# spiraldb/vortex

Hardware: AMD Instinct MI355X
Metric: decoded GB/s/GPU (device-resident) per encoding; % HBM roofline (higher is better)
Workload: dtype u32

## Files before the change

### vortex_amd/csrc/capi.hip

```cpp
#include <algorithm>
#include <cstring>
#include <mutex>

#include "encode_gpu.hpp"
#include "planner.hpp"

namespace vxg {

const float kF10f[11] = {1.0f, 10.0f, 100.0f, 1000.0f, 10000.0f, 100000.0f, 1000000.0f,
                         10000000.0f, 100000000.0f, 1000000000.0f, 10000000000.0f};
const float kIF10f[11] = {1.0f, 0.1f, 0.01f, 0.001f, 0.0001f, 0.00001f, 0.000001f,
                          0.0000001f, 0.00000001f, 0.000000001f, 0.0000000001f};
const double kF10d[24] = {
    1.0, 10.0, 100.0, 1000.0, 10000.0, 100000.0, 1000000.0, 10000000.0, 100000000.0,
    1000000000.0, 10000000000.0, 100000000000.0, 1000000000000.0, 10000000000000.0,
    100000000000000.0, 1000000000000000.0, 10000000000000000.0, 100000000000000000.0,
    1000000000000000000.0, 10000000000000000000.0, 100000000000000000000.0,
    1000000000000000000000.0, 10000000000000000000000.0, 100000000000000000000000.0};
const double kIF10d[24] = {
    1.0, 0.1, 0.01, 0.001, 0.0001, 0.00001, 0.000001, 0.0000001, 0.00000001, 0.000000001,
    0.0000000001, 0.00000000001, 0.000000000001, 0.0000000000001, 0.00000000000001,
    0.000000000000001, 0.0000000000000001, 0.00000000000000001, 0.000000000000000001,
    0.0000000000000000001, 0.00000000000000000001, 0.000000000000000000001,
    0.0000000000000000000001, 0.00000000000000000000001};
// ... 94 lines not shown
}

vxg_status vxg_set_option(vxg_ctx* ctx, int option, int64_t value) {
    if (!ctx) return set_error(VXG_ERR_INVALID_ARGUMENT, "null vxg_ctx");
    Options& o = ctx->c.opt;
    switch (option) {
    case VXG_OPT_K1W_MIN_GROUPS:
        if (value < 0 || value > (int64_t(1) << 31)) return set_error(VXG_ERR_INVALID_ARGUMENT, "K1W_MIN_GROUPS out of range");
        o.k1w_min_groups = value;
        return VXG_OK;
    case VXG_OPT_K1W_BPW:
        if (value < 0 || value > 32) return set_error(VXG_ERR_INVALID_ARGUMENT, "K1W_BPW must be in [0, 32]");
        o.k1w_bpw = value;
        return VXG_OK;
    case VXG_OPT_K1_WAVE:
        if (value < -1 || value > 2) return set_error(VXG_ERR_INVALID_ARGUMENT, "K1_WAVE must be -1, 0, 1 or 2");
        o.k1_wave = value;
        return VXG_OK;
    }
    return set_error(VXG_ERR_INVALID_ARGUMENT, "unknown option " + std::to_string(option));
}

vxg_status vxg_get_option(vxg_ctx* ctx, int option, int64_t* value) {
    if (!ctx || !value) return set_error(VXG_ERR_INVALID_ARGUMENT, "null argument");
    const Options& o = ctx->c.opt;
    switch (option) {
    case VXG_OPT_K1W_MIN_GROUPS: *value = o.k1w_min_groups; return VXG_OK;
    case VXG_OPT_K1W_BPW: *value = o.k1w_bpw; return VXG_OK;
    case VXG_OPT_K1_WAVE: *value = o.k1_wave; return VXG_OK;
    }
    return set_error(VXG_ERR_INVALID_ARGUMENT, "unknown option " + std::to_string(option));
}

vxg_status vxg_get_launch_stats(vxg_ctx* ctx, vxg_launch_stats* out, int reset) {
    if (!ctx || !out) return set_error(VXG_ERR_INVALID_ARGUMENT, "null argument");
    std::lock_guard<std::mutex> lk(ctx->c.mu);
    const LaunchStats& st = ctx->c.st;
    *out = vxg_launch_stats{};
    out->k1w_launches = st.k1w_launches;
    out->k1w_last_groups = st.k1w_last_groups;
    out->k1w_last_bpw = st.k1w_last_bpw;
    out->k1w_min_bpw = st.k1w_min_bpw;
    out->k1w_max_bpw = st.k1w_max_bpw;
    out->k1w_last_bpw_max = st.k1w_last_bpw_max;
    if (reset) ctx->c.st = LaunchStats{};
    return VXG_OK;
}

vxg_status vxg_close(vxg_ctx* ctx) {
    if (!ctx) return VXG_OK;
    if (g_cur_ctx == &ctx->c) g_cur_ctx = nullptr;
    (void)hipSetDevice(ctx->c.device);
    (void)hipDeviceSynchronize();
    if (ctx->c.err_word) (void)hipFree(ctx->c.err_word);
    delete ctx;
    return VXG_OK;
}

vxg_status vxg_alloc(vxg_ctx* ctx, uint64_t bytes, void** dptr) {
    VXG_TRY(use_device(ctx));
    return hip_check(hipMalloc(dptr, bytes ? bytes : 16), "hipMalloc");
}

vxg_status vxg_free(vxg_ctx* ctx, void* dptr) {
    VXG_TRY(use_device(ctx));
    return hip_check(hipFree(dptr), "hipFree");
}

vxg_status vxg_host_alloc(vxg_ctx* ctx, uint64_t bytes, void** hptr) {
    VXG_TRY(use_device(ctx));
    return hip_check(hipHostMalloc(hptr, bytes ? bytes : 16, hipHostMallocDefault), "hipHostMalloc");
}

vxg_status vxg_host_free(vxg_ctx* ctx, void* hptr) {
    VXG_TRY(use_device(ctx));
    return hip_check(hipHostFree(hptr), "hipHostFree");
}

vxg_status vxg_memcpy_h2d(vxg_ctx* ctx, void* dst, const void* src, uint64_t bytes, void* stream) {
    VXG_TRY(use_device(ctx));
    return hip_check(hipMemcpyAsync(dst, src, bytes, hipMemcpyHostToDevice, S(stream)), "h2d");
}

vxg_status vxg_memcpy_d2h(vxg_ctx* ctx, void* dst, const void* src, uint64_t bytes, void* stream) {
    VXG_TRY(use_device(ctx));
    return hip_check(hipMemcpyAsync(dst, src, bytes, hipMemcpyDeviceToHost, S(stream)), "d2h");
}

vxg_status vxg_memcpy_d2d(vxg_ctx* ctx, void* dst, const void* src, uint64_t bytes, void* stream) {
    VXG_TRY(use_device(ctx));
    return hip_check(hipMemcpyAsync(dst, src, bytes, hipMemcpyDeviceToDevice, S(stream)), "d2d");
}

vxg_status vxg_stream_sync(vxg_ctx* ctx, void* stream) {
    VXG_TRY(use_device(ctx));
    VXG_TRY(hip_check(hipStreamSynchronize(S(stream)), "hipStreamSynchronize"));
    uint32_t err = 0;
    VXG_TRY(hip_check(hipMemcpy(&err, ctx->c.err_word, 4, hipMemcpyDeviceToHost), "error word readback"));
    if (err) {
        VXG_TRY(hip_check(hipMemset(ctx->c.err_word, 0, 4), "error word reset"));
        return status_of_err_word(err);
    }
    return VXG_OK;
}

vxg_status vxg_canonical_size(vxg_ctx* ctx, const vxg_array* a, uint64_t* values_bytes, uint64_t* data_bytes) {
// ... 500 lines not shown
```

### vortex_amd/csrc/plan.hip

```cpp
#include <algorithm>
#include <chrono>
#include <cstdio>
#include <memory>

#include "k1g.hpp"
#include "planner.hpp"

using namespace vxg;

static uint64_t tree_bytes(const vxg_array& a) {
    uint64_t b = 0;
    for (uint32_t i = 0; i < a.n_buffers; i++) b += a.buffers[i].len;
    for (uint32_t i = 0; i < a.n_children; i++) b += tree_bytes(a.children[i]);
    return b;
}

static uint16_t leading_encoding(const vxg_array& a) {
    return a.encoding == VXG_ENC_CHUNKED && a.n_children ? leading_encoding(a.children[0]) : a.encoding;
}

static uint64_t canonical_out_bytes(const vxg_array& a) {
    return a.dtype == VXG_DTYPE_BOOL ? a.len / 8 : a.len * (is_string(a) ? 16 : ptype_width(a.ptype));
}

// ... 10 lines not shown
}

enum class BatchMode { Auto, Off, On, Mixed, Strings };
static BatchMode plan_batch_mode() {
    const char* e = env_str("VXG_PLAN_BATCH");
    if (!e || !*e) return BatchMode::Auto;
    if (e[0] == '0') return BatchMode::Off;
    if (e[0] == '1') return BatchMode::On;
    if (e[0] == 'm') return BatchMode::Mixed;
    if (e[0] == 's') return BatchMode::Strings;
    return BatchMode::Auto;
}
static bool dict_string_column(const vxg_array& a) {
    if (!is_string(a)) return false;
    if (a.encoding == VXG_ENC_CHUNKED) {
        for (uint32_t i = 1; i < a.n_children; i++)
            if (a.children[i].encoding != VXG_ENC_DICT) return false;
        return a.n_children > 1;
    }
    return a.encoding == VXG_ENC_DICT;
}
static uint64_t plan_batch_max_bytes() { return env_u64("VXG_PLAN_BATCH_MAX_BYTES", uint64_t(64) << 20); }

struct FusedNode {
    FsstFusedArgs fa;
    const GenChunk* gtab;
    uint32_t gn, dict_off;
    bool dict_lds;
    uint32_t* err;
    uint64_t gpe;
    void* args[7];
    hipGraphNode_t node = nullptr;
    hipKernelNodeParams p{};
    explicit FusedNode(void** a) {
        fa = *static_cast<const FsstFusedArgs*>(a[0]);
        gtab = *static_cast<const GenChunk* const*>(a[1]);
        gn = *static_cast<const uint32_t*>(a[2]);
        dict_off = *static_cast<const uint32_t*>(a[3]);
        dict_lds = *static_cast<const bool*>(a[4]);
        err = *static_cast<uint32_t* const*>(a[5]);
        gpe = *static_cast<const uint64_t*>(a[6]);
        void* const mine[7] = {&fa, &gtab, &gn, &dict_off, &dict_lds, &err, &gpe};
        std::copy(mine, mine + 7, args);
    }
};

struct vxg_plan {
    vxg_ctx* ctx = nullptr;
    std::vector<std::unique_ptr<FusedNode>> fused;
    uint64_t launches = 0;
    hipGraph_t graph = nullptr;
    hipGraphExec_t exec = nullptr;
    DevTables store;
    std::vector<hipKernelNodeParams> direct;
    bool batched = false;
    uint32_t branches = 0;
    vxg_plan_info info{};
};

static size_t plan_direct_max() { return size_t(env_u64("VXG_PLAN_DIRECT_MAX", 16)); }
static bool plan_direct_enabled() { return env_flag("VXG_PLAN_DIRECT", true); }

static std::vector<hipKernelNodeParams> kernel_chain(hipGraph_t g) {
    std::vector<hipKernelNodeParams> out;
    size_t nn = 0;
    if (hipGraphGetNodes(g, nullptr, &nn) != hipSuccess || nn == 0 || nn > plan_direct_max()) return out;
    std::vector<hipGraphNode_t> nodes(nn);
    if (hipGraphGetNodes(g, nodes.data(), &nn) != hipSuccess) return out;
    std::vector<hipGraphNode_t> dep(nn, nullptr);
    size_t roots = 0, root = 0;
    for (size_t i = 0; i < nn; i++) {
        hipGraphNodeType t{};
        if (hipGraphNodeGetType(nodes[i], &t) != hipSuccess || t != hipGraphNodeTypeKernel) {
            if (env_str("VXG_PLAN_DEBUG")) std::fprintf(stderr, "plan: node %zu of %zu has type %d\n", i, nn, int(t));
            return out;
        }
        size_t nd = 0;
        if (hipGraphNodeGetDependencies(nodes[i], nullptr, &nd) != hipSuccess || nd > 1) return out;
        if (nd == 1 && hipGraphNodeGetDependencies(nodes[i], &dep[i], &nd) != hipSuccess) return out;
        if (nd == 0) {
            roots++;
            root = i;
        }
    }
    if (roots != 1) return out;
    std::vector<size_t> order{root};
    while (order.size() < nn) {
        size_t next = nn, cnt = 0;
        for (size_t i = 0; i < nn; i++)
            if (dep[i] == nodes[order.back()]) {
                next = i;
                cnt++;
            }
        if (cnt != 1) return out;
        order.push_back(next);
    }
    for (size_t i : order) {
        hipKernelNodeParams p{};
        if (hipGraphKernelNodeGetParams(nodes[i], &p) != hipSuccess || p.extra || !p.kernelParams || !p.func) {
            out.clear();
            return out;
        }
        out.push_back(p);
    }
    return out;
}

static vxg_status bind_fused_nodes(vxg_plan* pl, hipGraph_t g) {
    size_t nn = 0;
    if (hipGraphGetNodes(g, nullptr, &nn) != hipSuccess) return set_error(VXG_ERR_ASSERTION_FAILED, "graph nodes");
    std::vector<hipGraphNode_t> nodes(nn);
    if (nn && hipGraphGetNodes(g, nodes.data(), &nn) != hipSuccess) return set_error(VXG_ERR_ASSERTION_FAILED, "graph nodes");
    for (hipGraphNode_t nd : nodes) {
        hipGraphNodeType t{};
        if (hipGraphNodeGetType(nd, &t) != hipSuccess || t != hipGraphNodeTypeKernel) continue;
        hipKernelNodeParams p{};
        if (hipGraphKernelNodeGetParams(nd, &p) != hipSuccess || !p.kernelParams || !is_fsst_fused_kernel(p.func)) continue;
        if (static_cast<const FsstFusedArgs*>(p.kernelParams[0])->prepass == 0) continue;
        auto f = std::make_unique<FusedNode>(p.kernelParams);
        f->node = nd;
        f->p = p;
        f->p.kernelParams = f->args;
        for (hipKernelNodeParams& d : pl->direct)
            if (d.func == p.func) d.kernelParams = f->args;
        pl->fused.push_back(std::move(f));
    }
    return VXG_OK;
}

static vxg_status record_plan(vxg_ctx* ctx, const vxg_array* arrays, vxg_canonical* outs, uint32_t n,
                              const std::vector<bool>& batched, uint32_t branches, vxg_plan** plan) {
    *plan = nullptr;
    const bool batching = std::find(batched.begin(), batched.end(), true) != batched.end();
    const bool own = batching && branches > 1;
    const uint32_t nb = (n < branches ? (n ? n : 1) : branches) + (own ? 1 : 0);
    const uint32_t na = own ? nb - 1 : nb;
    PlanBatch batch;
    hipStream_t cs;
    VXG_TRY(hip_check(hipStreamCreateWithFlags(&cs, hipStreamNonBlocking), "plan stream"));
    std::vector<hipStream_t> br(nb, nullptr);
    std::vector<hipEvent_t> ev(nb + 1, nullptr);
    vxg_status st = VXG_OK;
    for (uint32_t b = 0; b < nb && st == VXG_OK; b++)
        st = hip_check(hipStreamCreateWithFlags(&br[b], hipStreamNonBlocking), "plan branch stream");
    for (uint32_t b = 0; b <= nb && st == VXG_OK; b++)
        st = hip_check(hipEventCreateWithFlags(&ev[b], hipEventDisableTiming), "plan event");
    auto* pl = new vxg_plan();
    pl->ctx = ctx;
    pl->batched = batching;
    pl->branches = na;
    if (st == VXG_OK) st = hip_check(hipStreamBeginCapture(cs, hipStreamCaptureModeRelaxed), "hipStreamBeginCapture");
    if (st == VXG_OK) {
        st = hip_check(hipEventRecord(ev[nb], cs), "fork");
        for (uint32_t b = 0; b < nb && st == VXG_OK; b++)
            st = hip_check(hipStreamWaitEvent(br[b], ev[nb], 0), "fork wait");
        std::vector<uint32_t> order(n);
        std::vector<uint64_t> cost(n), load(na, 0);
        for (uint32_t i = 0; i < n; i++) {
            order[i] = i;
            cost[i] = plan_cost(arrays[i]);
        }
        std::stable_sort(order.begin(), order.end(), [&](uint32_t x, uint32_t y) { return cost[x] > cost[y]; });
        for (uint32_t k = 0; k < n && st == VXG_OK; k++) {
            const uint32_t i = order[k];
            const uint32_t b = uint32_t(std::min_element(load.begin(), load.end()) - load.begin());
            if (!(own && batched[i])) load[b] += cost[i];
            Planner p(ctx, br[b], &pl->store, batched[i] ? &batch : nullptr);
            st = p.canonical(arrays[i], outs[i]);
        }
        for (uint32_t b = 0; own && b < na && st == VXG_OK; b++) {
            st = hip_check(hipEventRecord(ev[b], br[b]), "batch join");
            if (st == VXG_OK) st = hip_check(hipStreamWaitEvent(br[nb - 1], ev[b], 0), "batch join wait");
        }
        if (batching && st == VXG_OK) st = flush_plan_batch(batch, ctx->c.err_word, br[nb - 1], &pl->store);
        for (uint32_t b = 0; b < nb && st == VXG_OK; b++) {
            st = hip_check(hipEventRecord(ev[b], br[b]), "join");
            if (st == VXG_OK) st = hip_check(hipStreamWaitEvent(cs, ev[b], 0), "join wait");
        }
        hipGraph_t g = nullptr;
        const hipError_t e = hipStreamEndCapture(cs, &g);
        if (st == VXG_OK) st = hip_check(e, "hipStreamEndCapture");
        pl->graph = g;
        if (st == VXG_OK && env_str("VXG_PLAN_DOT")) {
            static int cnt = 0;
            const std::string path = std::string(env_str("VXG_PLAN_DOT")) + "_" + std::to_string(cnt++) + ".dot";
            (void)hipGraphDebugDotPrint(g, path.c_str(), 0);
        }
        if (st == VXG_OK)
            st = hip_check(hipGraphInstantiate(&pl->exec, g, nullptr, nullptr, 0), "hipGraphInstantiate");
        if (st == VXG_OK) st = pl->store.upload();
        if (st == VXG_OK && plan_direct_enabled()) pl->direct = kernel_chain(g);
        if (st == VXG_OK) st = bind_fused_nodes(pl, g);
    }
    for (hipEvent_t e : ev)
        if (e) (void)hipEventDestroy(e);
    for (hipStream_t b : br)
        if (b) (void)hipStreamDestroy(b);
    (void)hipStreamDestroy(cs);
    if (st == VXG_OK) *plan = pl;
    else vxg_plan_destroy(pl);
    return st;
}

static vxg_status time_plans(const std::vector<vxg_plan*>& cands, int reps, std::vector<float>* ms) {
    hipStream_t s;
    VXG_TRY(hip_check(hipStreamCreateWithFlags(&s, hipStreamNonBlocking), "plan timing stream"));
    hipEvent_t e0 = nullptr, e1 = nullptr;
    vxg_status st = hip_check(hipEventCreate(&e0), "plan timing event");
    if (st == VXG_OK) st = hip_check(hipEventCreate(&e1), "plan timing event");
    std::vector<std::vector<float>> t(cands.size());
    for (vxg_plan* p : cands)
        if (st == VXG_OK) st = vxg_plan_launch(p, s);
    for (int r = 0; r < reps && st == VXG_OK; r++) {
        for (size_t c = 0; c < cands.size() && st == VXG_OK; c++) {
            st = hip_check(hipEventRecord(e0, s), "plan timing");
            if (st == VXG_OK) st = vxg_plan_launch(cands[c], s);
            if (st == VXG_OK) st = hip_check(hipEventRecord(e1, s), "plan timing");
            if (st == VXG_OK) st = hip_check(hipEventSynchronize(e1), "plan timing");
            float x = 0;
            if (st == VXG_OK) st = hip_check(hipEventElapsedTime(&x, e0, e1), "plan timing");
            t[c].push_back(x);
        }
    }
    if (e0) (void)hipEventDestroy(e0);
    if (e1) (void)hipEventDestroy(e1);
    (void)hipStreamSynchronize(s);
    (void)hipStreamDestroy(s);
    ms->clear();
    for (auto& v : t) {
        std::sort(v.begin(), v.end());
        ms->push_back(v.empty() ? 0.f : v[v.size() / 2]);
    }
    return st;
}

static uint32_t graph_cost(hipGraph_t g) {
    size_t nn = 0, ne = 0;
    if (!g || hipGraphGetNodes(g, nullptr, &nn) != hipSuccess) return 0;
    if (hipGraphGetEdges(g, nullptr, nullptr, &ne) != hipSuccess) ne = 0;
    return uint32_t(nn + ne);
}

extern "C" {

uint32_t vxg_plan_select(const float* ms, const uint32_t* cost, uint32_t n, uint32_t* selection) {
    uint32_t sel = VXG_PLAN_SEL_SINGLE, best = 0;
    if (n > 1 && !ms) {
        sel = VXG_PLAN_SEL_UNMEASURED;
        for (uint32_t c = 1; c < n; c++)
            if (cost && cost[c] < cost[best]) best = c;
    } else if (n > 1) {
// ... 72 lines not shown
    for (size_t c = 0; c < plans.size(); c++) cost[c] = graph_cost(plans[c]->graph);
    if (st == VXG_OK && measure && plans.size() > 1) {
        st = hip_check(hipDeviceSynchronize(), "plan create: device synchronize");
        uint32_t pending = 0;
        if (st == VXG_OK)
            st = hip_check(hipMemcpy(&pending, ctx->c.err_word, 4, hipMemcpyDeviceToHost), "error word readback");
        if (st == VXG_OK && pending) {
            best = vxg_plan_select(nullptr, cost.data(), uint32_t(plans.size()), &selection);
        } else if (st == VXG_OK) {
            st = time_plans(plans, 3, &ms);
            if (st == VXG_OK) best = vxg_plan_select(ms.data(), cost.data(), uint32_t(plans.size()), &selection);
            if (st == VXG_OK) {
                uint32_t err = 0;
                st = hip_check(hipMemcpy(&err, ctx->c.err_word, 4, hipMemcpyDeviceToHost), "error word readback");
                if (st == VXG_OK && err) {
                    st = hip_check(hipMemset(ctx->c.err_word, 0, 4), "error word reset");
                    if (st == VXG_OK) st = status_of_err_word(err);
                }
            }
        }
        if (env_str("VXG_PLAN_DEBUG"))
            for (size_t c = 0; c < ms.size(); c++)
                std::fprintf(stderr, "plan candidate %zu (%s, %u branches, %zu kernel-chain nodes): %.4f ms%s\n", c,
                             plans[c]->batched ? "batched" : "unbatched", cand[c].second, plans[c]->direct.size(),
                             ms[c], c == best ? "  <- kept" : "");
    }
    if (st == VXG_OK && !plans.empty()) {
        vxg_plan_info& in = plans[best]->info;
        in.batched = plans[best]->batched;
        in.branches = plans[best]->branches;
        in.direct_nodes = uint32_t(plans[best]->direct.size());
        in.n_candidates = uint32_t(std::min<size_t>(plans.size(), 2));
        for (size_t c = 0; c < plans.size() && c < 2; c++) {
            in.candidate_batched[c] = plans[c]->batched;
            in.candidate_ms[c] = ms[c];
        }
        in.selection = selection;
        for (size_t c = 0; c < plans.size() && c < 2; c++) in.candidate_cost[c] = cost[c];
        in.create_ms = std::chrono::duration<float, std::milli>(std::chrono::steady_clock::now() - t0).count();
    }
    for (size_t c = 0; c < plans.size(); c++)
        if (st != VXG_OK || c != best) vxg_plan_destroy(plans[c]);
    if (st == VXG_OK && !plans.empty()) *plan = plans[best];
    return st;
}

vxg_status vxg_plan_get_info(const vxg_plan* plan, vxg_plan_info* info) {
    if (!plan || !info) return set_error(VXG_ERR_INVALID_ARGUMENT, "null plan/info");
    *info = plan->info;
    return VXG_OK;
}

vxg_status vxg_plan_launch(vxg_plan* plan, void* stream) {
    if (!plan || !plan->exec) return set_error(VXG_ERR_INVALID_ARGUMENT, "null plan");
    VXG_TRY(use_device(plan->ctx));
    const uint32_t tag = uint32_t(++plan->launches % 65535u) + 1u;
    for (auto& f : plan->fused) f->fa.tag = tag;
    if (!plan->direct.empty()) {
        for (const hipKernelNodeParams& p : plan->direct)
            VXG_TRY(hip_check(hipLaunchKernel(p.func, p.gridDim, p.blockDim, p.kernelParams, p.sharedMemBytes, S(stream)),
                              "plan kernel"));
        return VXG_OK;
    }
    for (auto& f : plan->fused)
        VXG_TRY(hip_check(hipGraphExecKernelNodeSetParams(plan->exec, f->node, &f->p), "plan fused launch tag"));
    return hip_check(hipGraphLaunch(plan->exec, S(stream)), "hipGraphLaunch");
}

vxg_status vxg_plan_destroy(vxg_plan* plan) {
    if (!plan) return VXG_OK;
    if (plan->ctx) (void)hipSetDevice(plan->ctx->c.device);
    if (plan->exec) (void)hipGraphExecDestroy(plan->exec);
    if (plan->graph) (void)hipGraphDestroy(plan->graph);
    if (!plan->store.allocs.empty()) (void)hipDeviceSynchronize();
    for (void* p : plan->store.allocs) (void)hipFree(p);
    delete plan;
    return VXG_OK;
}

}
```

### vortex_amd/csrc/planner.hpp

```cpp
#pragma once

#include <hip/hip_runtime.h>

#include <cstdint>
#include <string>
#include <utility>
#include <vector>

#include "compare.hpp"
#include "compare_str.hpp"
#include "env.hpp"
#include "k1g.hpp"
#include "take.hpp"
#include "take_str.hpp"
#include "vxg_internal.hpp"

struct vxg_ctx {
    vxg::Ctx c;
};

#define VXG_TRY(expr)                         \
    do {                                      \
        vxg_status _s = (expr);               \
        if (_s != VXG_OK) return _s;          \
    } while (0)

namespace vxg {

inline hipStream_t S(void* s) { return static_cast<hipStream_t>(s); }

vxg_status use_device(vxg_ctx* ctx);
vxg_status status_of_err_word(uint32_t err);

inline bool is_string(const vxg_array& a) { return a.dtype == VXG_DTYPE_UTF8 || a.dtype == VXG_DTYPE_BINARY; }

struct PlanBatch {
    struct Run {
        int w;
        RunEndChunk c;
        bool indep;
    };
    std::vector<VarBinChunk> dicts;
    std::vector<K1Job> jobs;
    std::vector<Run> runs;
    std::vector<FsstChunk> fssts;
    bool empty() const { return dicts.empty() && jobs.empty() && runs.empty() && fssts.empty(); }
};

vxg_status make_k1_job(int T, unsigned W, unsigned offset, uint64_t len, const void* packed, uint64_t packed_bytes,
                       Epi epi, int vw, const UnpackArgs& a, void* out, K1Job& j);
vxg_status launch_k1_jobs(std::vector<K1Job>& jobs, uint32_t* err, hipStream_t s, DevTables* dt, const PatchCol* patch);
vxg_status launch_runs(std::vector<RunEndChunk> runs, int w, uint32_t* err, hipStream_t s, DevTables* dt);
vxg_status launch_varbin_dicts(const std::vector<VarBinChunk>& dicts, uint32_t* err, hipStream_t s, DevTables* dt);
vxg_status flush_plan_batch(PlanBatch& b, uint32_t* err, hipStream_t s, DevTables* dt);

struct PatchJob {
    const vxg_array* sp;
    int T;
    Epi epi;
    int vw;
    UnpackArgs a;
    void* dst;
    uint64_t out_len;
};
struct K1Sink { std::vector<K1Job>& jobs; std::vector<PatchJob>& patches; };

class Planner {
  public:
    Planner(vxg_ctx* ctx, hipStream_t s, DevTables* plan = nullptr, PlanBatch* batch = nullptr)
        : ctx_(ctx), s_(s), plan_(plan), batch_(batch) {}
    ~Planner() {
        for (void* p : temps_) (void)hipFreeAsync(p, s_);
    }

    vxg_status canonical(const vxg_array& a, vxg_canonical& out);
    vxg_status take(const vxg_array& a, const void* idx, int iw, bool isg, uint64_t n, uint32_t flags, vxg_canonical& out,
                    vxg_take_info& info);
    vxg_status filter(const vxg_array& a, const vxg_array& pred, vxg_canonical& out);
    vxg_status compare(const vxg_array& a, int op, uint64_t scalar_bits, uint32_t flags, vxg_canonical& out,
                       vxg_compare_info& info);
    vxg_status compare_bytes(const vxg_array& a, int op, const void* scalar_host, uint64_t scalar_len, uint32_t flags,
                             vxg_canonical& out, vxg_compare_bytes_info& info);
    vxg_status row_filter(const vxg_predicate* preds, uint32_t n_preds, uint32_t flags, vxg_canonical& out,
                          uint64_t* count_dev, vxg_row_filter_info& info);
    vxg_status canonical_size(const vxg_array& a, uint64_t& vb, uint64_t& db);
    vxg_status string_layout(const vxg_array& a, std::vector<vxg_data_buffer>& bufs, uint64_t& extent);
    static vxg_status string_buffer_count(const vxg_array& a, uint32_t& n);

  private:
    vxg_ctx* ctx_;
    hipStream_t s_;
    std::vector<void*> temps_;
    DevTables* plan_ = nullptr;
    PlanBatch* batch_ = nullptr;
    const vxg_array* root_ = nullptr;
    bool defer(const vxg_array& a) const { return batch_ && &a == root_; }
    bool k1_fusable(const vxg_array& c) const;

    vxg_status temp(uint64_t bytes, void** p) {
        if (bytes == 0) bytes = 16;
        if (plan_) {
            VXG_TRY(hip_check(hipMalloc(p, (bytes + 15) & ~15ull), "hipMalloc (plan temporary)"));
            plan_->allocs.push_back(*p);
            return VXG_OK;
        }
        VXG_TRY(hip_check(hipMallocAsync(p, (bytes + 15) & ~15ull, s_), "hipMallocAsync"));
        temps_.push_back(*p);
        return VXG_OK;
    }

    static bool is_primitive_dtype(const vxg_array& a) { return a.dtype == VXG_DTYPE_PRIMITIVE; }
    static int width(const vxg_array& a) { return ptype_width(a.ptype); }

    const vxg_buffer* buf(const vxg_array& a, uint32_t i) const {
        return i < a.n_buffers ? &a.buffers[i] : nullptr;
    }
    const vxg_array* child(const vxg_array& a, uint32_t i) const {
        return i < a.n_children ? &a.children[i] : nullptr;
    }

    vxg_status decode_into(const vxg_array& a, void* dst, K1Sink* sink = nullptr);
    vxg_status view_primitive(const vxg_array& a, const void** p);
    vxg_status int_column(const vxg_array& a, IntCol& c);
    vxg_status packed_column(const vxg_array& a, IntCol& c, bool* packed);
    vxg_status runend_column(const vxg_array& a, bool in_place, IntCol& c);

    vxg_status describe_bitpacked(const vxg_array& bp, Epi epi, int vw, UnpackArgs& a, void* dst, K1Job& j,
                                  const vxg_array** patches);
    vxg_status submit_k1(const K1Job& j, const vxg_array* patches, const UnpackArgs& a, K1Sink* sink, const PatchCol* fused);
    vxg_status decode_bitpacked(const vxg_array& bp, Epi epi, int vw, UnpackArgs a, void* dst, K1Sink* sink);
    bool patch_fusable(const vxg_array& sparse, int value_width) const;
    vxg_status sparse_patch_col(const vxg_array& sparse, PatchCol& pc);
    vxg_status apply_sparse_patches(const vxg_array& sparse, int T, Epi epi, int vw, const UnpackArgs& a,
                                    void* dst, uint64_t out_len);
    vxg_status decode_alp(const vxg_array& a, void* dst, K1Sink* sink);
    vxg_status decode_dict_primitive(const vxg_array& a, void* dst, K1Sink* sink);
    vxg_status decode_chunked_primitive(const vxg_array& a, void* dst);
    vxg_status decode_alprd(const vxg_array& a, void* dst);
    vxg_status decode_sparse_values(const vxg_array& a, void* dst);

    vxg_take_info* tinfo_ = nullptr;
    vxg_status take_values(const vxg_array& a, const void* idx, int iw, bool isg, uint64_t n, void* dst);
    vxg_status take_codes(const vxg_array& codes, const void* idx, int iw, bool isg, uint64_t n, void* dst);
    vxg_status take_validity(const vxg_array& a, const void* idx, int iw, bool isg, uint64_t n, vxg_canonical& out);
    vxg_status take_strings(const vxg_array& a, const void* idx, int iw, bool isg, uint64_t n, bool force,
                            vxg_canonical& out, vxg_take_info& info);
    vxg_status take_patches(const vxg_array& sp, TakePatches& p);
    struct CmpFused {
        const vxg_array* arr;
        const vxg_array* bp;
        const vxg_array* outer;
        int T, ck;
        Epi epi;
        EpiParams ep;
        CmpChunk d;
        bool excl;
    };
    vxg_status compare_shape(const vxg_array& a, uint64_t out_bit, CmpFused& f, bool* fused);
// ... 24 lines not shown
```

### vortex_amd/csrc/planner_launch.hip

```cpp
#include <algorithm>
#include <tuple>

#include "chunk_pack.hpp"
#include "k1g.hpp"
#include "planner.hpp"

static_assert(sizeof(vxg::ChunkTable) <= 4096, "ChunkTable exceeds the kernarg limit");
static_assert(sizeof(vxg::FsstTable) <= 4096, "FsstTable exceeds the kernarg limit");
static_assert(sizeof(vxg::RunEndTable) <= 4096, "RunEndTable exceeds the kernarg limit");
static_assert(sizeof(vxg::VarBinTable) <= 4096, "VarBinTable exceeds the kernarg limit");
static_assert(sizeof(vxg::CmpTable) + 32 <= 4096, "CmpTable and the compare arguments exceed the kernarg limit");

namespace vxg {

void note_k1w_launch(uint32_t bpw, uint32_t bpw_max, uint64_t groups) {
    if (!g_cur_ctx) return;
    std::lock_guard<std::mutex> lk(g_cur_ctx->mu);
    LaunchStats& st = g_cur_ctx->st;
    st.k1w_min_bpw = st.k1w_launches == 0 ? bpw : std::min(st.k1w_min_bpw, bpw);
    st.k1w_max_bpw = st.k1w_launches == 0 ? bpw : std::max(st.k1w_max_bpw, bpw);
    st.k1w_launches++;
    st.k1w_last_bpw = bpw;
    st.k1w_last_bpw_max = bpw_max;
    st.k1w_last_groups = groups;
// ... 130 lines not shown
    j.d.len = len;
    j.d.reference = a.reference;
    j.d.alp_a = a.alp_a;
    j.d.alp_b = a.alp_b;
    j.d.dict = a.dict;
    j.d.dict_len = a.dict_len;
    j.d.offset = offset;
    j.d.shift = a.shift;
    return VXG_OK;
}

vxg_status launch_runs(std::vector<RunEndChunk> runs, int w, uint32_t* err, hipStream_t s, DevTables* dt) {
    runs.erase(std::remove_if(runs.begin(), runs.end(), [](const RunEndChunk& r) { return r.len == 0; }), runs.end());
    std::vector<RunEndChunk> short_runs, long_runs;
    for (const RunEndChunk& r : runs) (r.len <= kRunEndShortRun * r.n_runs ? short_runs : long_runs).push_back(r);
    for (int pass = 0; pass < 2; pass++) {
        const std::vector<RunEndChunk>& rs = pass == 0 ? short_runs : long_runs;
        for (const RunEndChunk* it = rs.data(), * const end = rs.data() + rs.size(); it != end;) {
            RunEndTable tab{};
            tab.err = err;
            uint64_t groups;
            VXG_TRY(pack_chunk_table(
                tab, it, end, dt, [](const RunEndChunk& r) { return &r; },
                [pass](const RunEndChunk& r) {
                    return pass == 0 ? (r.n_runs + kRunEndRunsPerGroup - 1) / kRunEndRunsPerGroup
                                     : (r.len + kRunEndSpan - 1) / kRunEndSpan;
                },
                &groups));
            VXG_TRY(pass == 0 ? launch_runend_runs(w, tab, groups, s) : launch_runend_chunks(w, tab, groups, s));
        }
    }
    return VXG_OK;
}

static bool plan_fuse_enabled() { return env_flag("VXG_PLAN_FUSE", true); }

vxg_status launch_varbin_dicts(const std::vector<VarBinChunk>& dicts, uint32_t* err, hipStream_t s, DevTables* dt) {
    for (const VarBinChunk* it = dicts.data(), * const end = dicts.data() + dicts.size(); it != end;) {
        VarBinTable tab{};
        tab.err = err;
        uint64_t groups;
        VXG_TRY(pack_chunk_table(
            tab, it, end, dt, [](const VarBinChunk& d) { return &d; },
            [](const VarBinChunk& d) { return d.n ? (d.n + 255) / 256 : uint64_t(1); }, &groups));
        VXG_TRY(launch_varbin_chunks(tab, groups, s));
    }
    return VXG_OK;
}

vxg_status flush_plan_batch(PlanBatch& b, uint32_t* err, hipStream_t s, DevTables* dt) {
    FsstFused ff;
    if (!b.fssts.empty()) {
        void* scratch = nullptr;
        VXG_TRY(hip_check(hipMalloc(&scratch, (fsst_chunks_scratch_bytes(b.fssts.data(), b.fssts.size()) + 15) & ~15ull),
                            "hipMalloc (plan FSST scratch)"));
        dt->allocs.push_back(scratch);
        VXG_TRY(launch_fsst_batch(b.fssts, scratch, err, s, dt, plan_fuse_enabled() ? &ff : nullptr));
    }
    VXG_TRY(launch_varbin_dicts(b.dicts, err, s, dt));
    std::vector<std::pair<int, RunEndChunk>> gen_runs;
    std::vector<PlanBatch::Run> rest;
    for (const PlanBatch::Run& r : b.runs) {
        if (r.c.len == 0) continue;
        if (r.indep && r.c.len <= kRunEndShortRun * r.c.n_runs && gen_runs_kind(r.w) >= 0) gen_runs.emplace_back(r.w, r.c);
        else rest.push_back(r);
    }
    VXG_TRY(launch_plan_k1_jobs(b.jobs, gen_runs, ff, err, s, *dt));
    std::vector<int> widths;
    for (const auto& r : rest) widths.push_back(r.w);
    std::sort(widths.begin(), widths.end());
    widths.erase(std::unique(widths.begin(), widths.end()), widths.end());
    for (int w : widths) {
        std::vector<RunEndChunk> rs;
        for (const auto& r : rest)
            if (r.w == w) rs.push_back(r.c);
        VXG_TRY(launch_runs(rs, w, err, s, dt));
    }
    return VXG_OK;
}

}
```

### vortex_amd/csrc/vxg_internal.hpp

```cpp
#pragma once

#include <hip/hip_runtime.h>

#include <cstdint>
#include <mutex>
#include <string>
#include <type_traits>
#include <vector>

#include "../../include/vortex_gpu.h"
#include "env.hpp"

namespace vxg {

__host__ __device__ constexpr int fl_order(int i) {
    constexpr int o[8] = {0, 4, 2, 6, 1, 5, 3, 7};
    return o[i];
}
__host__ __device__ constexpr int fl_index(int row, int lane) {
    return fl_order(row / 8) * 16 + (row % 8) * 128 + lane;
}

template <class T>
using gptr = __attribute__((address_space(1))) T*;
template <class T>
__device__ __forceinline__ T gload(const T* p) {
    if constexpr (sizeof(T) == 16 && !std::is_scalar_v<T>) {
        using u32x4 = unsigned int __attribute__((ext_vector_type(4)));
        const u32x4 x = *(gptr<const u32x4>)p;
        T r;
        __builtin_memcpy(&r, &x, 16);
        return r;
    } else {
        return *(gptr<const T>)p;
    }
}
template <class T>
__device__ __forceinline__ void gstore(T* p, const T& v) {
    if constexpr (sizeof(T) == 16 && !std::is_scalar_v<T>) {
        using u32x4 = unsigned int __attribute__((ext_vector_type(4)));
        u32x4 x;
        __builtin_memcpy(&x, &v, 16);
        *(gptr<u32x4>)p = x;
    } else {
        *(gptr<T>)p = v;
    }
}
template <class T>
__device__ __forceinline__ T lds_load(const T* p) {
    if constexpr (sizeof(T) == 16 && !std::is_scalar_v<T>) {
        using u32x4 = unsigned int __attribute__((ext_vector_type(4)));
        const u32x4 x = *(__attribute__((address_space(3))) const u32x4*)p;
        T r;
        __builtin_memcpy(&r, &x, 16);
        return r;
    } else {
        return *(__attribute__((address_space(3))) const T*)p;
    }
}

template <typename V>
__device__ __forceinline__ void nt_store(V* p, const V& v) {
    if constexpr (sizeof(V) == 16) {
        using u32x4 = unsigned int __attribute__((ext_vector_type(4)));
// ... 9 lines not shown
    switch (p) {
    case VXG_U8: case VXG_I8: return 1;
    case VXG_U16: case VXG_I16: case VXG_F16: return 2;
    case VXG_U32: case VXG_I32: case VXG_F32: return 4;
    case VXG_U64: case VXG_I64: case VXG_F64: return 8;
    default: return 0;
    }
}
inline bool ptype_is_int(int p) { return p >= VXG_U8 && p <= VXG_I64; }
inline bool ptype_is_signed(int p) { return p >= VXG_I8 && p <= VXG_I64; }
inline bool ptype_is_unsigned(int p) { return p >= VXG_U8 && p <= VXG_U64; }

extern const float kF10f[11];
extern const float kIF10f[11];
extern const double kF10d[24];
extern const double kIF10d[24];

enum : uint32_t { kErrTakeOOB = 1u, kErrPatchOOB = 2u, kErrRunEnd = 4u, kErrFsst = 8u, kErrRoaring = 16u, kErrVarBin = 32u,
                  kErrPatchOrder = 64u, kErrPlanSync = 128u };

struct Options {
    int64_t k1w_min_groups = 1024;
    int64_t k1w_bpw = 0;
    int64_t k1_wave = -1;
};
struct LaunchStats {
    uint64_t k1w_launches = 0, k1w_last_groups = 0;
    uint32_t k1w_last_bpw = 0, k1w_min_bpw = 0, k1w_max_bpw = 0, k1w_last_bpw_max = 0;
};

struct Ctx {
    int device = 0;
    uint32_t* err_word = nullptr;
    Options opt;
    std::mutex mu;
    LaunchStats st;
};
extern thread_local Ctx* g_cur_ctx;
Options default_options();
inline Options cur_options() { return g_cur_ctx ? g_cur_ctx->opt : default_options(); }
inline int k1_wave_mode() {
    const int64_t o = cur_options().k1_wave;
    if (o >= 0) return int(o > 2 ? 2 : o);
    const char* e = env_str("VXG_K1_WAVE");
    if (!e) return 1;
    return e[0] == '0' ? 0 : (e[0] == 'f' ? 2 : 1);
}
void note_k1w_launch(uint32_t bpw, uint32_t bpw_max, uint64_t groups);

vxg_status set_error(vxg_status s, const std::string& msg);
vxg_status hip_check(hipError_t e, const char* what);

struct DevTables {
    std::vector<void*> allocs;
    std::vector<std::pair<void*, std::vector<uint8_t>>> uploads;
    template <class E>
    vxg_status table(size_t n, E** host, const E** dev) {
        void* d = nullptr;
        const hipError_t e = hipMalloc(&d, n * sizeof(E) + 16);
        if (e != hipSuccess) return hip_check(e, "hipMalloc (plan chunk table)");
        allocs.push_back(d);
        uploads.emplace_back(d, std::vector<uint8_t>(n * sizeof(E), 0));
        *host = reinterpret_cast<E*>(uploads.back().second.data());
        *dev = static_cast<const E*>(d);
        return VXG_OK;
    }
    vxg_status upload() {
        for (auto& u : uploads) {
            const hipError_t e = hipMemcpy(u.first, u.second.data(), u.second.size(), hipMemcpyHostToDevice);
            if (e != hipSuccess) return hip_check(e, "plan chunk table upload");
        }
        uploads.clear();
        return VXG_OK;
    }
};

template <class E, class Key>
__device__ __forceinline__ uint32_t ext_chunk_index(const E* __restrict__ ext, uint32_t n, uint64_t g, Key key) {
    const uint32_t lane = threadIdx.x & 63u;
    uint32_t cnt = 0;
    for (uint32_t base = 0; base < n; base += 256) {
        uint64_t kv[4];
#pragma unroll
        for (int k = 0; k < 4; k++) {
            const uint32_t i = base + 64u * uint32_t(k) + lane;
            kv[k] = uint64_t(key(ext[i < n ? i : n - 1]));
        }
#pragma unroll
        for (int k = 0; k < 4; k++) {
            const bool le = base + 64u * uint32_t(k) + lane < n && kv[k] <= g;
            cnt += uint32_t(__popcll(__ballot(le)));
        }
    }
    return cnt ? cnt - 1 : 0;
}

template <class E, class Key>
__device__ __forceinline__ uint32_t ext_chunk_index_gpe(const E* __restrict__ ext, uint32_t n, uint64_t g, uint64_t gpe,
                                                        Key key) {
    if (gpe) {
        const uint32_t q = uint32_t(g) / uint32_t(gpe);
        const uint32_t ci = __builtin_amdgcn_readfirstlane(q < n - 1 ? q : n - 1);
        const uint64_t f0 = uint64_t(key(ext[ci]));
        const uint64_t f1 = ci + 1 < n ? uint64_t(key(ext[ci + 1])) : ~0ull;
        if (f0 <= g && g < f1) return ci;
    }
    return ext_chunk_index(ext, n, g, key);
}
inline uint64_t common_groups(const uint64_t* counts, size_t n) {
    if (n == 0 || counts[0] == 0) return 0;
    for (size_t i = 1; i + 1 < n; i++)
        if (counts[i] != counts[0]) return 0;
    return counts[n - 1] <= counts[0] ? counts[0] : 0;
}

enum class Epi : int { Plain = 0, For = 1, ForZigZag = 2, AlpF32 = 3, AlpF64 = 4, Dict = 5 };

struct UnpackArgs {
    const uint8_t* packed;
    void* out;
    uint64_t n_blocks;
    uint32_t offset;
    uint64_t len;
    uint64_t reference;
    uint32_t shift;
// ... 213 lines not shown
```

Baseline: 4839.

## Pool plan allocations in an arena and cache capture streams and events

Plan recording now bump-allocates chunk tables and scratch from a per-context arena backed by a reusable block cache, replacing one hipMalloc per table and per temporary. Tables are uploaded with one memcpy per block. Capture streams and events are cached on the context instead of being created and destroyed for every plan, and graph instantiation is skipped when the direct kernel chain is used. This targets plan creation overhead rather than the decode kernels, at the cost of more retained device memory and added phase-timing debug code.

```diff
diff --git a/vortex_amd/csrc/capi.hip b/vortex_amd/csrc/capi.hip
--- a/vortex_amd/csrc/capi.hip
+++ b/vortex_amd/csrc/capi.hip
@@ -170,6 +170,8 @@
     if (g_cur_ctx == &ctx->c) g_cur_ctx = nullptr;
     (void)hipSetDevice(ctx->c.device);
     (void)hipDeviceSynchronize();
+    ctx->plan_rec.destroy();
+    ctx->plan_blocks.free_all();
     if (ctx->c.err_word) (void)hipFree(ctx->c.err_word);
     delete ctx;
     return VXG_OK;
diff --git a/vortex_amd/csrc/plan.hip b/vortex_amd/csrc/plan.hip
--- a/vortex_amd/csrc/plan.hip
+++ b/vortex_amd/csrc/plan.hip
@@ -86,6 +86,7 @@
     hipGraph_t graph = nullptr;
     hipGraphExec_t exec = nullptr;
     DevTables store;
+    explicit vxg_plan(vxg_ctx* c) : ctx(c), store(&c->plan_blocks) {}
     std::vector<hipKernelNodeParams> direct;
     bool batched = false;
     uint32_t branches = 0;
@@ -162,6 +163,92 @@
     return VXG_OK;
 }
 
+namespace vxg {
+
+bool PlanBlockCache::acquire(size_t bytes, ArenaBlock* out) {
+    {
+        std::lock_guard<std::mutex> lk(*mu);
+        for (size_t i = 0; i < free_list.size(); i++) {
+            if (free_list[i].bytes != bytes) continue;
+            *out = free_list[i];
+            free_list[i] = free_list.back();
+            free_list.pop_back();
+            free_bytes -= bytes;
+            reused++;
+            return true;
+        }
+    }
+    void* d = nullptr;
+    if (hipMalloc(&d, bytes) != hipSuccess) {
+        (void)hipGetLastError();
+        free_all();
+        if (hipMalloc(&d, bytes) != hipSuccess) {
+            (void)hipGetLastError();
+            return false;
+        }
+    }
+    std::lock_guard<std::mutex> lk(*mu);
+    fresh++;
+    *out = ArenaBlock{d, bytes};
+    return true;
+}
+
+void PlanBlockCache::release(const ArenaBlock& b) {
+    std::vector<ArenaBlock> drop;
+    {
+        std::lock_guard<std::mutex> lk(*mu);
+        free_list.push_back(b);
+        free_bytes += b.bytes;
+        while (free_list.size() > kPlanCacheBlocks || free_bytes > kPlanCacheBytes) {
+            const auto big = std::max_element(free_list.begin(), free_list.end(),
+                                              [](const ArenaBlock& x, const ArenaBlock& y) { return x.bytes < y.bytes; });
+            drop.push_back(*big);
+            free_bytes -= big->bytes;
+            *big = free_list.back();
+            free_list.pop_back();
+        }
+    }
+    for (const ArenaBlock& d : drop) (void)hipFree(d.dev);
+}
+
+void PlanBlockCache::free_all() {
+    std::vector<ArenaBlock> drop;
+    {
+        std::lock_guard<std::mutex> lk(*mu);
+        drop.swap(free_list);
+        free_bytes = 0;
+    }
+    for (const ArenaBlock& b : drop) (void)hipFree(b.dev);
+}
+
+void PlanRecordObjects::destroy() {
+    for (hipEvent_t e : ev)
+        if (e) (void)hipEventDestroy(e);
+    for (hipStream_t b : br)
+        if (b) (void)hipStreamDestroy(b);
+    if (cs) (void)hipStreamDestroy(cs);
+    ev.clear();
+    br.clear();
+    cs = nullptr;
+}
+
+}
+
+static vxg_status ensure_record_objects(PlanRecordObjects& o, uint32_t nb) {
+    if (!o.cs) VXG_TRY(hip_check(hipStreamCreateWithFlags(&o.cs, hipStreamNonBlocking), "plan stream"));
+    while (o.br.size() < nb) {
+        hipStream_t s = nullptr;
+        VXG_TRY(hip_check(hipStreamCreateWithFlags(&s, hipStreamNonBlocking), "plan branch stream"));
+        o.br.push_back(s);
+    }
+    while (o.ev.size() < size_t(nb) + 1) {
+        hipEvent_t e = nullptr;
+        VXG_TRY(hip_check(hipEventCreateWithFlags(&e, hipEventDisableTiming), "plan event"));
+        o.ev.push_back(e);
+    }
+    return VXG_OK;
+}
+
 static vxg_status record_plan(vxg_ctx* ctx, const vxg_array* arrays, vxg_canonical* outs, uint32_t n,
                               const std::vector<bool>& batched, uint32_t branches, vxg_plan** plan) {
     *plan = nullptr;
@@ -170,19 +257,27 @@
     const uint32_t nb = (n < branches ? (n ? n : 1) : branches) + (own ? 1 : 0);
     const uint32_t na = own ? nb - 1 : nb;
     PlanBatch batch;
-    hipStream_t cs;
-    VXG_TRY(hip_check(hipStreamCreateWithFlags(&cs, hipStreamNonBlocking), "plan stream"));
-    std::vector<hipStream_t> br(nb, nullptr);
-    std::vector<hipEvent_t> ev(nb + 1, nullptr);
-    vxg_status st = VXG_OK;
-    for (uint32_t b = 0; b < nb && st == VXG_OK; b++)
-        st = hip_check(hipStreamCreateWithFlags(&br[b], hipStreamNonBlocking), "plan branch stream");
-    for (uint32_t b = 0; b <= nb && st == VXG_OK; b++)
-        st = hip_check(hipEventCreateWithFlags(&ev[b], hipEventDisableTiming), "plan event");
-    auto* pl = new vxg_plan();
-    pl->ctx = ctx;
+    using clk = std::chrono::steady_clock;
+    const auto ms_since = [](clk::time_point a) { return std::chrono::duration<double, std::milli>(clk::now() - a).count(); };
+    double ph[5] = {0, 0, 0, 0, 0};
+    auto tp = clk::now();
+    PlanRecordObjects mine;
+    bool cached;
+    {
+        std::lock_guard<std::mutex> lk(ctx->c.mu);
+        cached = !ctx->plan_rec.busy;
+        if (cached) ctx->plan_rec.busy = true;
+    }
+    PlanRecordObjects& ro = cached ? ctx->plan_rec : mine;
+    vxg_status st = ensure_record_objects(ro, nb);
+    const hipStream_t cs = ro.cs;
+    const std::vector<hipStream_t>& br = ro.br;
+    const std::vector<hipEvent_t>& ev = ro.ev;
+    auto* pl = new vxg_plan(ctx);
     pl->batched = batching;
     pl->branches = na;
+    ph[0] = ms_since(tp);
+    tp = clk::now();
     if (st == VXG_OK) st = hip_check(hipStreamBeginCapture(cs, hipStreamCaptureModeRelaxed), "hipStreamBeginCapture");
     if (st == VXG_OK) {
         st = hip_check(hipEventRecord(ev[nb], cs), "fork");
@@ -215,22 +310,53 @@
         const hipError_t e = hipStreamEndCapture(cs, &g);
         if (st == VXG_OK) st = hip_check(e, "hipStreamEndCapture");
         pl->graph = g;
+        ph[1] = ms_since(tp);
         if (st == VXG_OK && env_str("VXG_PLAN_DOT")) {
             static int cnt = 0;
             const std::string path = std::string(env_str("VXG_PLAN_DOT")) + "_" + std::to_string(cnt++) + ".dot";
             (void)hipGraphDebugDotPrint(g, path.c_str(), 0);
         }
-        if (st == VXG_OK)
-            st = hip_check(hipGraphInstantiate(&pl->exec, g, nullptr, nullptr, 0), "hipGraphInstantiate");
-        if (st == VXG_OK) st = pl->store.upload();
+        tp = clk::now();
         if (st == VXG_OK && plan_direct_enabled()) pl->direct = kernel_chain(g);
         if (st == VXG_OK) st = bind_fused_nodes(pl, g);
-    }
-    for (hipEvent_t e : ev)
-        if (e) (void)hipEventDestroy(e);
-    for (hipStream_t b : br)
-        if (b) (void)hipStreamDestroy(b);
-    (void)hipStreamDestroy(cs);
+        ph[4] = ms_since(tp);
+        tp = clk::now();
+        if (st == VXG_OK && pl->direct.empty())
+            st = hip_check(hipGraphInstantiate(&pl->exec, g, nullptr, nullptr, 0), "hipGraphInstantiate");
+        ph[2] = ms_since(tp);
+        tp = clk::now();
+        if (st == VXG_OK) st = pl->store.upload();
+        ph[3] = ms_since(tp);
+        if (env_str("VXG_PLAN_DEBUG")) {
+            const PlanArena& ar = pl->store.arena;
+            uint64_t fresh, reused;
+            size_t cache_blocks, cache_bytes;
+            {
+                std::lock_guard<std::mutex> lk(ctx->c.mu);
+                fresh = ctx->plan_blocks.fresh;
+                reused = ctx->plan_blocks.reused;
+                cache_blocks = ctx->plan_blocks.free_list.size();
+                cache_bytes = ctx->plan_blocks.free_bytes;
+            }
+            std::fprintf(stderr,
+                         "plan phases ms: streams_events %.4f capture %.4f instantiate %.4f upload %.4f chain_bind %.4f | "
+                         "arena blocks=%zu table_blocks=%zu footprint_bytes=%zu used_bytes=%zu table_bytes=%zu "
+                         "allocations=%zu uploads=%u | context blocks fresh=%llu reused=%llu cached=%zu cached_bytes=%zu "
+                         "streams_cached=%d | %s, %u branches, %zu chain nodes, exec=%d\n",
+                         ph[0], ph[1], ph[2], ph[3], ph[4], ar.n_blocks(), ar.n_blocks(PlanArena::Tables), ar.reserved_bytes(),
+                         ar.used_bytes(), ar.table_bytes(), ar.n_allocations(), pl->store.n_uploads,
+                         static_cast<unsigned long long>(fresh), static_cast<unsigned long long>(reused), cache_blocks,
+                         cache_bytes, int(cached), batching ? "batched" : "unbatched", na, pl->direct.size(),
+                         int(pl->exec != nullptr));
+        }
+    }
+    if (!cached) {
+        mine.destroy();
+    } else {
+        if (st != VXG_OK) ro.destroy();
+        std::lock_guard<std::mutex> lk(ctx->c.mu);
+        ctx->plan_rec.busy = false;
+    }
     if (st == VXG_OK) *plan = pl;
     else vxg_plan_destroy(pl);
     return st;
@@ -409,7 +535,7 @@
 }
 
 vxg_status vxg_plan_launch(vxg_plan* plan, void* stream) {
-    if (!plan || !plan->exec) return set_error(VXG_ERR_INVALID_ARGUMENT, "null plan");
+    if (!plan || (!plan->exec && plan->direct.empty())) return set_error(VXG_ERR_INVALID_ARGUMENT, "null plan");
     VXG_TRY(use_device(plan->ctx));
     const uint32_t tag = uint32_t(++plan->launches % 65535u) + 1u;
     for (auto& f : plan->fused) f->fa.tag = tag;
@@ -429,8 +555,7 @@
     if (plan->ctx) (void)hipSetDevice(plan->ctx->c.device);
     if (plan->exec) (void)hipGraphExecDestroy(plan->exec);
     if (plan->graph) (void)hipGraphDestroy(plan->graph);
-    if (!plan->store.allocs.empty()) (void)hipDeviceSynchronize();
-    for (void* p : plan->store.allocs) (void)hipFree(p);
+    if (plan->store.arena.n_blocks()) (void)hipDeviceSynchronize();
     delete plan;
     return VXG_OK;
 }
diff --git a/vortex_amd/csrc/plan_arena.hpp b/vortex_amd/csrc/plan_arena.hpp
--- /dev/null
+++ b/vortex_amd/csrc/plan_arena.hpp
@@ -0,0 +1,136 @@
+#pragma once
+
+#include <cstddef>
+#include <cstdint>
+#include <cstdlib>
+#include <cstring>
+#include <memory>
+#include <vector>
+
+namespace vxg {
+
+struct ArenaBlock {
+    void* dev = nullptr;
+    size_t bytes = 0;
+};
+
+struct ArenaSource {
+    virtual ~ArenaSource() = default;
+    virtual bool acquire(size_t bytes, ArenaBlock* out) = 0;
+    virtual void release(const ArenaBlock& b) = 0;
+};
+
+class PlanArena {
+  public:
+    static constexpr size_t kAlign = 256;
+    static constexpr size_t kFirstBlock = 64u << 10;
+    static constexpr size_t kGrowth = 4;
+    static constexpr size_t kMaxClass = 64u << 20;
+    static constexpr size_t kOversizeAlign = 2u << 20;
+    static constexpr size_t kTail = kAlign;
+
+    enum Region { Tables = 0, Scratch = 1 };
+
+    explicit PlanArena(ArenaSource* src) : src_(src) {}
+    PlanArena(const PlanArena&) = delete;
+    PlanArena& operator=(const PlanArena&) = delete;
+    ~PlanArena() { release(); }
+
+    static size_t block_bytes(size_t need, size_t last) {
+        need += kTail;
+        size_t b = last ? (last >= kMaxClass ? kMaxClass : last * kGrowth) : kFirstBlock;
+        while (b < need && b < kMaxClass) b *= kGrowth;
+        if (b < need) b = (need + kOversizeAlign - 1) / kOversizeAlign * kOversizeAlign;
+        return b;
+    }
+
+    void* table(size_t bytes, void** host) {
+        Blk* b = nullptr;
+        size_t off = 0;
+        if (!bump(Tables, bytes, &b, &off)) return nullptr;
+        *host = b->mirror.get() + off;
+        return static_cast<uint8_t*>(b->blk.dev) + off;
+    }
+    void* scratch(size_t bytes) {
+        Blk* b = nullptr;
+        size_t off = 0;
+        if (!bump(Scratch, bytes, &b, &off)) return nullptr;
+        return static_cast<uint8_t*>(b->blk.dev) + off;
+    }
+
+    template <class Copy>
+    bool upload(Copy copy) const {
+        for (const Blk& b : blocks_[Tables])
+            if (b.used && !copy(b.blk.dev, static_cast<const void*>(b.mirror.get()), b.used)) return false;
+        return true;
+    }
+    void drop_mirrors() {
+        for (Blk& b : blocks_[Tables]) b.mirror.reset();
+    }
+
+    void release() {
+        for (auto& r : blocks_) {
+            for (Blk& b : r) src_->release(b.blk);
+            r.clear();
+        }
+    }
+
+    size_t n_blocks() const { return blocks_[Tables].size() + blocks_[Scratch].size(); }
+    size_t n_blocks(Region r) const { return blocks_[r].size(); }
+    size_t n_allocations() const { return n_allocs_; }
+    size_t reserved_bytes() const { return sum([](const Blk& b) { return b.blk.bytes; }); }
+    size_t used_bytes() const { return sum([](const Blk& b) { return b.used; }); }
+    size_t table_bytes() const {
+        size_t t = 0;
+        for (const Blk& b : blocks_[Tables]) t += b.used;
+        return t;
+    }
+    const ArenaBlock& block(Region r, size_t i) const { return blocks_[r][i].blk; }
+
+  private:
+    struct FreeDeleter {
+        void operator()(uint8_t* p) const { std::free(p); }
+    };
+    struct Blk {
+        ArenaBlock blk;
+        size_t used = 0;
+        std::unique_ptr<uint8_t, FreeDeleter> mirror;
+    };
+
+    bool bump(Region r, size_t bytes, Blk** out, size_t* off) {
+        if (bytes > SIZE_MAX / 2) return false;
+        const size_t need = (bytes ? bytes + kAlign - 1 : kAlign) / kAlign * kAlign;
+        std::vector<Blk>& bs = blocks_[r];
+        if (bs.empty() || bs.back().used + need + kTail > bs.back().blk.bytes) {
+            Blk nb;
+            if (!src_->acquire(block_bytes(need, bs.empty() ? 0 : bs.back().blk.bytes), &nb.blk)) return false;
+            if (r == Tables) {
+                nb.mirror.reset(static_cast<uint8_t*>(std::calloc(nb.blk.bytes, 1)));
+                if (!nb.mirror) {
+                    src_->release(nb.blk);
+                    return false;
+                }
+            }
+            bs.push_back(std::move(nb));
+        }
+        Blk& b = bs.back();
+        *out = &b;
+        *off = b.used;
+        b.used += need;
+        n_allocs_++;
+        return true;
+    }
+    template <class F>
+    size_t sum(F f) const {
+        size_t t = 0;
+        for (const auto& r : blocks_)
+            for (const Blk& b : r) t += f(b);
+        return t;
+    }
+
+    ArenaSource* src_;
+    std::vector<Blk> blocks_[2];
+    size_t n_allocs_ = 0;
+};
+
+}
diff --git a/vortex_amd/csrc/planner.hpp b/vortex_amd/csrc/planner.hpp
--- a/vortex_amd/csrc/planner.hpp
+++ b/vortex_amd/csrc/planner.hpp
@@ -15,8 +15,34 @@
 #include "take_str.hpp"
 #include "vxg_internal.hpp"
 
+namespace vxg {
+
+constexpr size_t kPlanCacheBytes = size_t(192) << 20;
+constexpr size_t kPlanCacheBlocks = 64;
+struct PlanBlockCache final : ArenaSource {
+    std::mutex* mu = nullptr;
+    std::vector<ArenaBlock> free_list;
+    size_t free_bytes = 0;
+    uint64_t fresh = 0, reused = 0;
+    bool acquire(size_t bytes, ArenaBlock* out) override;
+    void release(const ArenaBlock& b) override;
+    void free_all();
+};
+struct PlanRecordObjects {
+    bool busy = false;
+    hipStream_t cs = nullptr;
+    std::vector<hipStream_t> br;
+    std::vector<hipEvent_t> ev;
+    void destroy();
+};
+
+}
+
 struct vxg_ctx {
     vxg::Ctx c;
+    vxg::PlanBlockCache plan_blocks;
+    vxg::PlanRecordObjects plan_rec;
+    vxg_ctx() { plan_blocks.mu = &c.mu; }
 };
 
 #define VXG_TRY(expr)                         \
@@ -99,11 +125,7 @@
 
     vxg_status temp(uint64_t bytes, void** p) {
         if (bytes == 0) bytes = 16;
-        if (plan_) {
-            VXG_TRY(hip_check(hipMalloc(p, (bytes + 15) & ~15ull), "hipMalloc (plan temporary)"));
-            plan_->allocs.push_back(*p);
-            return VXG_OK;
-        }
+        if (plan_) return plan_->scratch(bytes, p);
         VXG_TRY(hip_check(hipMallocAsync(p, (bytes + 15) & ~15ull, s_), "hipMallocAsync"));
         temps_.push_back(*p);
         return VXG_OK;
diff --git a/vortex_amd/csrc/planner_launch.hip b/vortex_amd/csrc/planner_launch.hip
--- a/vortex_amd/csrc/planner_launch.hip
+++ b/vortex_amd/csrc/planner_launch.hip
@@ -206,9 +206,7 @@
     FsstFused ff;
     if (!b.fssts.empty()) {
         void* scratch = nullptr;
-        VXG_TRY(hip_check(hipMalloc(&scratch, (fsst_chunks_scratch_bytes(b.fssts.data(), b.fssts.size()) + 15) & ~15ull),
-                            "hipMalloc (plan FSST scratch)"));
-        dt->allocs.push_back(scratch);
+        VXG_TRY(dt->scratch(fsst_chunks_scratch_bytes(b.fssts.data(), b.fssts.size()), &scratch));
         VXG_TRY(launch_fsst_batch(b.fssts, scratch, err, s, dt, plan_fuse_enabled() ? &ff : nullptr));
     }
     VXG_TRY(launch_varbin_dicts(b.dicts, err, s, dt));
diff --git a/vortex_amd/csrc/vxg_internal.hpp b/vortex_amd/csrc/vxg_internal.hpp
--- a/vortex_amd/csrc/vxg_internal.hpp
+++ b/vortex_amd/csrc/vxg_internal.hpp
@@ -10,6 +10,7 @@
 
 #include "../../include/vortex_gpu.h"
 #include "env.hpp"
+#include "plan_arena.hpp"
 
 namespace vxg {
 
@@ -125,25 +126,31 @@
 vxg_status hip_check(hipError_t e, const char* what);
 
 struct DevTables {
-    std::vector<void*> allocs;
-    std::vector<std::pair<void*, std::vector<uint8_t>>> uploads;
+    PlanArena arena;
+    uint32_t n_uploads = 0;
+    explicit DevTables(ArenaSource* blocks) : arena(blocks) {}
     template <class E>
     vxg_status table(size_t n, E** host, const E** dev) {
-        void* d = nullptr;
-        const hipError_t e = hipMalloc(&d, n * sizeof(E) + 16);
-        if (e != hipSuccess) return hip_check(e, "hipMalloc (plan chunk table)");
-        allocs.push_back(d);
-        uploads.emplace_back(d, std::vector<uint8_t>(n * sizeof(E), 0));
-        *host = reinterpret_cast<E*>(uploads.back().second.data());
+        void* h = nullptr;
+        void* d = arena.table(n * sizeof(E) + 16, &h);
+        if (!d) return set_error(VXG_ERR_OUT_OF_MEMORY, "plan arena: out of memory (chunk table)");
+        *host = static_cast<E*>(h);
         *dev = static_cast<const E*>(d);
         return VXG_OK;
     }
+    vxg_status scratch(uint64_t bytes, void** p) {
+        *p = arena.scratch(size_t((bytes + 15) & ~15ull));
+        return *p ? VXG_OK : set_error(VXG_ERR_OUT_OF_MEMORY, "plan arena: out of memory (temporary)");
+    }
     vxg_status upload() {
-        for (auto& u : uploads) {
-            const hipError_t e = hipMemcpy(u.first, u.second.data(), u.second.size(), hipMemcpyHostToDevice);
-            if (e != hipSuccess) return hip_check(e, "plan chunk table upload");
-        }
-        uploads.clear();
+        hipError_t err = hipSuccess;
+        arena.upload([&](void* d, const void* h, size_t used) {
+            err = hipMemcpy(d, h, used, hipMemcpyHostToDevice);
+            n_uploads++;
+            return err == hipSuccess;
+        });
+        if (err != hipSuccess) return hip_check(err, "plan chunk table upload");
+        arena.drop_mirrors();
         return VXG_OK;
     }
 };
```

Result: no change. 4830 (-0.2%).
